# ShengkaiWu/IoU-aware-single-stage-object-detector

Measured on AMD Instinct MI355X. Metric: images/sec at 1333x800, IoU-aware RetinaNet R-50-FPN, higher is better.
Workload: dtype fp32; 1 GPU; IoU-aware RetinaNet R-50-FPN fp32, batch 8 per GPU, 3x800x1344 (1333x800 padded to /32), random-init weights, whole inference path incl. NMS, device-to-host copy and bbox2result (the reference's simple_test: per-class arrays on the host; batch i's host part runs under batch i+1's device part, the last one inside the timed region); global_batch=8, parallelism=dp1, dets_per_image=100

## Files before the change

### include/iouaware.h

```cpp
#ifndef IOUAWARE_H
#define IOUAWARE_H

#include <stddef.h>
#include <stdint.h>

#ifdef __cplusplus
extern "C" {
#endif

#define IA_MAX_LEVELS 8
#define IA_MAX_ANCHORS 16
#define IA_MAX_NMS_PRE 4096
#define IA_MAX_CANDIDATES 8192
#define IA_MAX_PER_IMG 1024

#define IA_F32 0
#define IA_BF16 1
#define IA_F16 2
#define IA_F64 3

#define IA_LAYOUT_NCHW 0
#define IA_LAYOUT_NHWC 1

#define IA_CLS_SIGMOID 0
// ... 120 lines not shown
    int32_t H[IA_MAX_LEVELS], W[IA_MAX_LEVELS];
} ia_wino_geom;
typedef struct {
    int32_t c0, n;
    int32_t dst_channels, dst_offset;
    float *dst[IA_MAX_LEVELS];
} ia_wino_seg;
int ia_wino_tiles(const ia_wino_geom *g, int32_t *tiles);
int ia_wino_input_transform(const ia_wino_geom *g, const float *const *x, int channels, int groups,
                            const float *pre_scale, const float *pre_shift, int pre_relu, float *V,
                            void *stream);
int ia_wino_output_transform(const ia_wino_geom *g, const float *M, int channels, int groups,
                             const float *bias, int relu, int nseg, const ia_wino_seg *segs,
                             void *stream);
int ia_wino_mid_transform(const ia_wino_geom *g, const float *M, int channels, int groups_m,
                          const float *bias, int relu, float *V, int groups_v, void *stream);
int ia_wino_in_gemm(const ia_wino_geom *g, const float *const *x, int channels, const float *pre_scale,
                    const float *pre_shift, int pre_relu, const float *u_packed, float *M, void *stream);
int ia_wino_conv3x3_c64(const ia_wino_geom *g, const float *const *x, int channels, const float *pre_scale,
                        const float *pre_shift, int pre_relu, const float *u_packed, const float *bias,
                        int relu, float *const *y, void *stream);

int ia_wino_grad_output_transform(const ia_wino_geom *g, const float *const *dy, int channels,
                                  float *dM, void *stream);

#define IA_COLSUM_MAX_STRIPS 512
size_t ia_relu_bwd_bias_grad_workspace_bytes(int64_t rows, int n);
int ia_wino_weight_transform(const float *w, int n_in, int n_out, int64_t stride_in,
                             int64_t stride_out, int64_t stride_ky, int64_t stride_kx, int flip,
                             const double *G, float *U, void *stream);
int ia_wino_weight_grad(const float *dU, int n_in, int n_out, const double *G, float *dW,
                        int64_t stride_in, int64_t stride_out, int64_t stride_ky, int64_t stride_kx,
                        void *stream);
int ia_bn_fold_fwd(const float *w, const float *gamma, const float *beta, const float *mean,
                   const float *inv_std, int cout, int K, float *w_out, float *b_out, void *stream);
int ia_bn_fold_bwd(const float *dw_folded, const float *db_folded, const float *w, const float *gamma,
                   const float *mean, const float *inv_std, int cout, int K, float *dw,
                   float *dgamma, float *dbeta, void *stream);
int ia_relu_bwd_bias_grad(const float *dy, const float *y, int64_t rows, int n, float *g, float *db,
                          void *workspace, size_t workspace_bytes, void *stream);

int ia_linear_bias_act(const float *A, const float *W, const float *bias, const float *residual,
                       float *D, int64_t rows, int k, int n, int relu, void *workspace,
                       size_t workspace_bytes, void *stream);
int ia_linear_bias_act_bf16(const void *A, const void *W, const float *bias, const void *residual,
                            void *D, int64_t rows, int k, int n, int relu, void *workspace,
                            size_t workspace_bytes, void *stream);
int ia_batched_gemm(const float *A, const float *W, float *D, int batch, int64_t rows, int k, int n,
                    void *workspace, size_t workspace_bytes, void *stream);
int ia_batched_gemm_stream(const float *A, const float *W, float *D, int batch, int64_t rows, int k,
                           int n, void *stream);
int ia_batched_gemm_split3(const float *V, const void *U3, float *D, int batch, int64_t rows, int k,
                           int n, void *stream);

size_t ia_im2col3x3_bytes(int B, int H, int W, int C, int stride, int dtype);
int ia_im2col3x3_nhwc(const void *x, void *col, int B, int H, int W, int C, int stride, int dtype,
                      void *stream);
int ia_conv1x1_strided(const void *x, const void *W_kn, const float *bias, const void *residual,
                       void *D, int B, int H, int W, int k, int n, int stride, int relu, int dtype,
                       void *workspace, size_t workspace_bytes, void *stream);
int ia_col2im3x3_nhwc(const void *dcol, void *dx, int B, int H, int W, int C, int stride, int dtype,
                      void *stream);

size_t ia_deform_im2col3x3_bytes(int B, int H, int W, int C, int stride, int pad, int dil);
int ia_deform_im2col3x3_nhwc(const float *x, const float *offset, int64_t offset_pix_stride,
                             const float *mask, int64_t mask_pix_stride, int mask_logits,
                             float *col, int B, int H, int W, int C, int stride, int pad,
                             int dil, int deformable_groups, void *stream);
int ia_deform_col2im3x3_nhwc(const float *dcol, const float *x, const float *offset,
                             int64_t offset_pix_stride, const float *mask,
                             int64_t mask_pix_stride, float *dx, float *d_offset, float *d_mask,
                             int B, int H, int W, int C, int stride, int pad, int dil,
                             int deformable_groups, void *stream);

int ia_gemm_tuning(int mode);

int ia_gemm_table_add(int64_t m, int64_t n, int64_t k, int flags, int batch, int dtype,
                      int solution_index);
int ia_gemm_table_clear(void);
int ia_gemm_table_dump(int64_t *rows7, int capacity);
int ia_gemm_table_stats(int64_t *hits_misses_stale);
int ia_gemm_library_version(void);

int ia_linear_bias_act_wt(const float *A, const float *W_nk, const float *bias,
                          const float *residual, float *D, int64_t rows, int k, int n, int relu,
                          void *workspace, size_t workspace_bytes, void *stream);
int ia_gemm_tn(const float *G, const float *X, float *D, int batch, int64_t rows, int n, int k,
               void *workspace, size_t workspace_bytes, void *stream);


int ia_focal_loss_fwd(const void *cls, int dtype, const int64_t *labels,
                      const float *label_weights, int B, int A, int C, int HW, float gamma,
                      float alpha, double *loss_sum, void *stream);
int ia_focal_loss_bwd(const void *cls, int dtype, const int64_t *labels,
                      const float *label_weights, int B, int A, int C, int HW, float gamma,
                      float alpha, float gscale, const float *gscale_dev, float *grad_cls,
                      void *stream);

int ia_smooth_l1_fwd(const void *pred, int dtype, const float *target, const float *weight,
                     int B, int A, int HW, float beta, double *loss_sum, void *stream);
int ia_smooth_l1_bwd(const void *pred, int dtype, const float *target, const float *weight,
                     int B, int A, int HW, float beta, float gscale, const float *gscale_dev,
                     float *grad_pred, void *stream);

int ia_balanced_l1_fwd(const void *pred, int dtype, const float *target, const float *weight,
                       int B, int A, int HW, float beta, float alpha, float gamma, double *loss_sum,
// ... 386 lines not shown
```

### iou-aware-single-stage-object-detector_amd/csrc/wino_split_gemm.hip

```cpp
#include "ia_internal.hpp"

namespace ia {

typedef __attribute__((ext_vector_type(8))) __bf16 bf16x8;
typedef __attribute__((ext_vector_type(16))) float f32x16;

constexpr int kSgBM = 128;
constexpr int kSgBN = 128;
constexpr int kSgBK = 32;
constexpr int kSgThreads = 256;
constexpr int kSgImg = 64 * 16;
constexpr int kSgStage = 2 * 4 * 3 * kSgImg;

struct SplitGemmArgs {
    const float *v;
    const uint4 *up;
    float *d;
    int64_t rows;
    int K, N, np32;
    int ntiles, mtiles;
};

__device__ __forceinline__ void split3(const float4 &x0, const float4 &x1, bf16x8 &h, bf16x8 &m, bf16x8 &l)
{
    const float x[8] = {x0.x, x0.y, x0.z, x0.w, x1.x, x1.y, x1.z, x1.w};
#pragma unroll
    for (int e = 0; e < 8; ++e) {
        const __bf16 hb = (__bf16)x[e];
        const float r = x[e] - (float)hb;
        const __bf16 mb = (__bf16)r;
        h[e] = hb;
        m[e] = mb;
        l[e] = (__bf16)(r - (float)mb);
    }
}

__global__ void __launch_bounds__(kSgThreads, 2) k_gemm_split3(SplitGemmArgs a)
{
    __shared__ __attribute__((aligned(16))) unsigned char s_a[kSgStage];
    __shared__ __attribute__((aligned(16))) unsigned char s_b[kSgStage];
    const int tid = threadIdx.x, lane = tid & 63, wv = tid >> 6;
    const int wm = wv >> 1, wn = wv & 1;
    int nt, b;
    int64_t row0;
    {
        const int total = (int)gridDim.x, q = total >> 3, r = total & 7;
        const int xcd = (int)blockIdx.x & 7, idx = (int)blockIdx.x >> 3;
        int t = xcd < r ? xcd * (q + 1) + idx : r * (q + 1) + (xcd - r) * q + idx;
        nt = t % a.ntiles;
        t /= a.ntiles;
        row0 = (int64_t)(t % a.mtiles) * kSgBM;
        b = t / a.mtiles;
    }
    const int nchunk = a.K / kSgBK;

    int64_t r = row0 + wv * 32 + (lane & 31);
    if (r >= a.rows) r = a.rows - 1;
    const float *vp = a.v + ((int64_t)b * a.rows + r) * a.K + 8 * (lane >> 5);
    const uint4 *up = a.up + ((int64_t)b * (a.K / 16) * a.np32 + nt * 4) * (3 * 64);
    const int64_t ks_stride = (int64_t)a.np32 * 3 * 64;

    float4 x0, x1, x2, x3;
    uint4 u0, u1, u2, u3, u4, u5;
#define SG_LOAD(c)                                                                                  \
    {                                                                                               \
        const float *src = vp + (c) * kSgBK;                                                        \
        x0 = *reinterpret_cast<const float4 *>(src);                                                \
        x1 = *reinterpret_cast<const float4 *>(src + 4);                                            \
        x2 = *reinterpret_cast<const float4 *>(src + 16);                                           \
        x3 = *reinterpret_cast<const float4 *>(src + 20);                                           \
        const uint4 *us = up + (int64_t)(2 * (c)) * ks_stride;                                      \
        u0 = us[tid];                                                                               \
        u1 = us[tid + 256];                                                                         \
// ... 54 lines not shown
                }
#pragma unroll
            for (int i = 0; i < 2; ++i)
#pragma unroll
                for (int j = 0; j < 2; ++j)
                    hi[i][j] = __builtin_amdgcn_mfma_f32_32x32x16_bf16(fa[i][0], fb[j][0], hi[i][j], 0, 0, 0);
#pragma unroll
            for (int i = 0; i < 2; ++i)
#pragma unroll
                for (int j = 0; j < 2; ++j)
                    lo[i][j] = __builtin_amdgcn_mfma_f32_32x32x16_bf16(fa[i][1], fb[j][1], lo[i][j], 0, 0, 0);
#pragma unroll
            for (int i = 0; i < 2; ++i)
#pragma unroll
                for (int j = 0; j < 2; ++j)
                    lo[i][j] = __builtin_amdgcn_mfma_f32_32x32x16_bf16(fa[i][0], fb[j][2], lo[i][j], 0, 0, 0);
#pragma unroll
            for (int i = 0; i < 2; ++i)
#pragma unroll
                for (int j = 0; j < 2; ++j)
                    lo[i][j] = __builtin_amdgcn_mfma_f32_32x32x16_bf16(fa[i][2], fb[j][0], lo[i][j], 0, 0, 0);
#pragma unroll
            for (int i = 0; i < 2; ++i)
#pragma unroll
                for (int j = 0; j < 2; ++j)
                    lo[i][j] = __builtin_amdgcn_mfma_f32_32x32x16_bf16(fa[i][0], fb[j][1], lo[i][j], 0, 0, 0);
#pragma unroll
            for (int i = 0; i < 2; ++i)
#pragma unroll
                for (int j = 0; j < 2; ++j)
                    lo[i][j] = __builtin_amdgcn_mfma_f32_32x32x16_bf16(fa[i][1], fb[j][0], lo[i][j], 0, 0, 0);
        }
    }
#undef SG_LOAD
#undef SG_STORE

    float *dst = a.d + (int64_t)b * a.rows * a.N;
#pragma unroll
    for (int j = 0; j < 2; ++j) {
        const int col = nt * kSgBN + wn * 64 + j * 32 + (lane & 31);
        if (col >= a.N) continue;
#pragma unroll
        for (int i = 0; i < 2; ++i) {
            const int64_t rb = row0 + wm * 64 + i * 32 + 4 * (lane >> 5);
#pragma unroll
            for (int e = 0; e < 16; ++e) {
                const int64_t row = rb + (e & 3) + 8 * (e >> 2);
                if (row < a.rows) dst[row * a.N + col] = hi[i][j][e] + lo[i][j][e];
            }
        }
    }
}

}

extern "C" int ia_batched_gemm_split3(const float *V, const void *U3, float *D, int batch, int64_t rows, int k,
                                      int n, void *stream)
{
    if (!V || !U3 || !D || rows < 1 || batch < 1 || batch > 65535 || k < ia::kSgBK || k % ia::kSgBK || n < 1)
        return IA_E_ARG;
    if (((uintptr_t)V & 15u) || ((uintptr_t)U3 & 15u) || ((uintptr_t)D & 3u)) return IA_E_ARG;
    const int64_t mt = (rows + ia::kSgBM - 1) / ia::kSgBM, ntiles = (n + ia::kSgBN - 1) / ia::kSgBN;
    if (mt * ntiles * batch > 2147483647LL) return IA_E_ARG;
    ia::SplitGemmArgs a;
    a.v = V; a.up = (const uint4 *)U3; a.d = D; a.rows = rows; a.K = k; a.N = n;
    a.np32 = (int)(ntiles * (ia::kSgBN / 32));
    a.ntiles = (int)ntiles; a.mtiles = (int)mt;
    const dim3 grid((unsigned)(mt * ntiles * batch)), block(ia::kSgThreads);
    hipLaunchKernelGGL(ia::k_gemm_split3, grid, block, 0, (hipStream_t)stream, a);
    return ia::hip_status(hipGetLastError());
}
```

### iou-aware-single-stage-object-detector_amd/iouaware/_lib.py

```python
import ctypes as C
import os

IA_MAX_LEVELS = 8
IA_MAX_ANCHORS = 16
IA_MAX_NMS_PRE = 4096
IA_MAX_CANDIDATES = 8192
IA_MAX_PER_IMG = 1024
IA_F32, IA_BF16, IA_F16, IA_F64 = 0, 1, 2, 3
IA_LAYOUT_NCHW, IA_LAYOUT_NHWC = 0, 1
IA_CLS_SIGMOID, IA_CLS_SOFTMAX = 0, 1
IA_CLS_SIGMOID_NOIOU, IA_CLS_SOFTMAX_NOIOU = 2, 3
IA_LOSS_SLOTS = 64
IA_MAX_TARGET_BATCH = 16
IA_GN_CHUNK = 256

_CSRC = os.path.join(os.path.dirname(os.path.abspath(__file__)), '..', 'csrc')
SO_PATH = os.path.abspath(os.path.join(_CSRC, 'libiouaware_hip.so'))


class HeadGeom(C.Structure):
    _fields_ = [('num_levels', C.c_int32), ('num_anchors', C.c_int32),
                ('num_classes', C.c_int32), ('nms_pre', C.c_int32),
                ('H', C.c_int32 * IA_MAX_LEVELS), ('W', C.c_int32 * IA_MAX_LEVELS),
                ('stride', C.c_int32 * IA_MAX_LEVELS),
# ... 110 lines not shown
    'ia_select_topk': (_i, [_G, _vp, _i, _vp, _vp, _sz, _vp]),
    'ia_decode_fuse_rowmax_grouped': (_i, [_G, _P, _i, _i, _vp, _vp, _sz, _vp]),
    'ia_select_topk_grouped': (_i, [_G, _vp, _i, _vp, _vp, _sz, _vp]),
    'ia_decode_stage': (_i, [_G, _P, _i, _i, _vp, _vp, _i, _vp, _sz, _vp]),
    'ia_get_bboxes_status_offset': (_sz, [_G, _i]),
    'ia_debug_fused_spin_limit': (_i, [_i64]),
    'ia_profile_stage_events': (_i, [_vp, _vp]),
    'ia_gather_decode': (_i, [_G, _P, _i, _i, _vp, _vp, _vp, _i, _vp, _vp, _vp, _vp]),
    'ia_multiclass_nms_workspace_bytes': (_sz, [_i, _i, _i]),
    'ia_multiclass_nms': (_i, [_vp, _vp, _vp, _i, _i, _i, _f, _f, _i, _vp, _sz, _vp, _vp, _vp,
                               _vp, _vp, _vp, _vp]),
    'ia_multiclass_soft_nms_workspace_bytes': (_sz, [_i, _i, _i]),
    'ia_multiclass_soft_nms': (_i, [_vp, _vp, _i, _i, _i, _f, _f, _i, _f, _f, _i, _vp, _sz, _vp, _vp,
                                    _vp, _vp, _vp, _vp, _vp]),
    'ia_soft_nms': (_i, [_vp, _i, _f, _i, _f, _f, _vp, _vp, _vp, _vp]),
    'ia_get_bboxes_workspace_bytes': (_sz, [_G, _i]),
    'ia_get_bboxes': (_i, [_G, _P, _i, _i, _vp, _vp, _i, _f, _f, _i, _vp, _sz, _vp, _vp, _vp,
                           _vp, _vp]),
    'ia_multiclass_nms_lazy_workspace_bytes': (_sz, [_i, _i, _i]),
    'ia_multiclass_nms_lazy': (_i, [_vp, _vp, _vp, _i, _i, _i, _f, _f, _i, _i, _vp, _sz, _vp, _vp, _vp,
                                    _vp, _vp]),
    'ia_get_bboxes_lazy': (_i, [_G, _P, _i, _i, _vp, _vp, _i, _f, _f, _i, _i, _vp, _sz, _vp, _vp, _vp,
                                _vp, _vp]),
    'ia_get_bboxes_workspace_layout': (_i, [_G, _i, C.POINTER(_sz * 8)]),
    'ia_nms_workspace_bytes': (_sz, [_i]),
    'ia_nms': (_i, [_vp, _i, _f, _vp, _vp, _vp, _sz, _vp]),
    'ia_nms_f64_workspace_bytes': (_sz, [_i]),
    'ia_nms_f64': (_i, [_vp, _i, _f, _vp, _vp, _vp, _sz, _vp]),
    'ia_image_transform': (_i, [C.POINTER(ImageDesc), _i, C.POINTER(C.c_float), C.POINTER(C.c_float),
                                _i, _i, _i, _i, _vp, _vp]),
    'ia_wino_tiles': (_i, [C.POINTER(WinoGeom), C.POINTER(C.c_int32)]),
    'ia_wino_input_transform': (_i, [C.POINTER(WinoGeom), C.POINTER(C.c_void_p), _i, _i, _vp, _vp, _i,
                                     _vp, _vp]),
    'ia_wino_grad_output_transform': (_i, [C.POINTER(WinoGeom), C.POINTER(C.c_void_p), _i, _vp, _vp]),
    'ia_wino_weight_transform': (_i, [_vp, _i, _i, C.c_int64, C.c_int64, C.c_int64, C.c_int64, _i,
                                      C.POINTER(C.c_double), _vp, _vp]),
    'ia_wino_weight_grad': (_i, [_vp, _i, _i, C.POINTER(C.c_double), _vp, C.c_int64, C.c_int64,
                                 C.c_int64, C.c_int64, _vp]),
    'ia_bn_fold_fwd': (_i, [_vp, _vp, _vp, _vp, _vp, _i, _i, _vp, _vp, _vp]),
    'ia_bn_fold_bwd': (_i, [_vp, _vp, _vp, _vp, _vp, _vp, _i, _i, _vp, _vp, _vp, _vp]),
    'ia_relu_bwd_bias_grad_workspace_bytes': (C.c_size_t, [C.c_int64, _i]),
    'ia_relu_bwd_bias_grad': (_i, [_vp, _vp, C.c_int64, _i, _vp, _vp, _vp, C.c_size_t, _vp]),
    'ia_wino_output_transform': (_i, [C.POINTER(WinoGeom), _vp, _i, _i, _vp, _i, _i,
                                      C.POINTER(WinoSeg), _vp]),
    'ia_wino_mid_transform': (_i, [C.POINTER(WinoGeom), _vp, _i, _i, _vp, _i, _vp, _i, _vp]),
    'ia_wino_in_gemm': (_i, [C.POINTER(WinoGeom), C.POINTER(C.c_void_p), _i, _vp, _vp, _i, _vp, _vp, _vp]),
    'ia_wino_conv3x3_c64': (_i, [C.POINTER(WinoGeom), C.POINTER(C.c_void_p), _i, _vp, _vp, _i, _vp, _vp, _i,
                                 C.POINTER(C.c_void_p), _vp]),
    'ia_linear_bias_act': (_i, [_vp, _vp, _vp, _vp, _vp, _i64, _i, _i, _i, _vp, _sz, _vp]),
    'ia_linear_bias_act_bf16': (_i, [_vp, _vp, _vp, _vp, _vp, _i64, _i, _i, _i, _vp, _sz, _vp]),
    'ia_batched_gemm': (_i, [_vp, _vp, _vp, _i, _i64, _i, _i, _vp, _sz, _vp]),
    'ia_batched_gemm_stream': (_i, [_vp, _vp, _vp, _i, _i64, _i, _i, _vp]),
    'ia_batched_gemm_split3': (_i, [_vp, _vp, _vp, _i, _i64, _i, _i, _vp]),
    'ia_linear_bias_act_wt': (_i, [_vp, _vp, _vp, _vp, _vp, _i64, _i, _i, _i, _vp, _sz, _vp]),
    'ia_gemm_tuning': (_i, [_i]),
    'ia_im2col3x3_bytes': (_sz, [_i, _i, _i, _i, _i, _i]),
    'ia_im2col3x3_nhwc': (_i, [_vp, _vp, _i, _i, _i, _i, _i, _i, _vp]),
    'ia_col2im3x3_nhwc': (_i, [_vp, _vp, _i, _i, _i, _i, _i, _i, _vp]),
    'ia_deform_im2col3x3_bytes': (_sz, [_i, _i, _i, _i, _i, _i, _i]),
    'ia_deform_im2col3x3_nhwc': (_i, [_vp, _vp, _i64, _vp, _i64, _i, _vp, _i, _i, _i, _i, _i, _i, _i, _i, _vp]),
    'ia_deform_col2im3x3_nhwc': (_i, [_vp, _vp, _vp, _i64, _vp, _i64, _vp, _vp, _vp, _i, _i, _i, _i, _i, _i,
                                      _i, _i, _vp]),
    'ia_conv1x1_strided': (_i, [_vp, _vp, _vp, _vp, _vp, _i, _i, _i, _i, _i, _i, _i, _i, _vp, _sz, _vp]),
    'ia_gemm_table_add': (_i, [_i64, _i64, _i64, _i, _i, _i, _i]),
    'ia_gemm_table_clear': (_i, []),
    'ia_gemm_table_dump': (_i, [_vp, _i]),
    'ia_gemm_table_stats': (_i, [_vp]),
    'ia_gemm_library_version': (_i, []),
    'ia_gemm_tn': (_i, [_vp, _vp, _vp, _i, _i64, _i, _i, _vp, _sz, _vp]),
    'ia_focal_loss_fwd': (_i, [_vp, _i, _vp, _vp, _i, _i, _i, _i, _f, _f, _vp, _vp]),
    'ia_focal_loss_bwd': (_i, [_vp, _i, _vp, _vp, _i, _i, _i, _i, _f, _f, _f, _vp, _vp, _vp]),
    'ia_smooth_l1_fwd': (_i, [_vp, _i, _vp, _vp, _i, _i, _i, _f, _vp, _vp]),
    'ia_smooth_l1_bwd': (_i, [_vp, _i, _vp, _vp, _i, _i, _i, _f, _f, _vp, _vp, _vp]),
    'ia_balanced_l1_fwd': (_i, [_vp, _i, _vp, _vp, _i, _i, _i, _f, _f, _f, _vp, _vp]),
    'ia_balanced_l1_bwd': (_i, [_vp, _i, _vp, _vp, _i, _i, _i, _f, _f, _f, _f, _vp, _vp, _vp]),
    'ia_focal_loss_balanced_fwd': (_i, [_vp, _i, _vp, _vp, _vp, _i, _i, _i, _i, _f, _f, _f, _vp, _vp]),
    'ia_focal_loss_balanced_bwd': (_i, [_vp, _i, _vp, _vp, _vp, _i, _i, _i, _i, _f, _f, _f, _vp, _f,
                                        _vp, _vp, _vp]),
    'ia_smooth_l1_balanced_fwd': (_i, [_vp, _i, _vp, _vp, _vp, _i, _i, _i, _f, _f, _vp, _vp]),
    'ia_smooth_l1_balanced_bwd': (_i, [_vp, _i, _vp, _vp, _vp, _i, _i, _i, _f, _f, _f, _vp, _vp,
                                       _vp]),
    'ia_iou_bce_fwd': (_i, [_G, _i, _vp, _vp, _i, _vp, _vp, _i, _vp, _vp, _vp]),
    'ia_iou_bce_bwd': (_i, [_G, _i, _vp, _vp, _i, _vp, _vp, _i, _f, _vp, _vp, _vp, _vp]),
    'ia_anchor_targets': (_i, [_G, _vp, _vp, _vp, _i, _i, _vp, _f, _f, _f, _f, _vp, _vp, _vp, _vp,
                               _vp, _vp, _vp]),
    'ia_anchor_targets_ptrs': (_i, [_G, C.POINTER(C.c_void_p), C.POINTER(C.c_void_p),
                                    C.POINTER(C.c_int32), _i, C.POINTER(C.c_int32), _f, _f, _f, _f,
                                    _vp, _vp, _vp, _vp, _vp, _vp, _vp]),
    'ia_head_loss_workspace_bytes': (_sz, [_G, _i]),
    'ia_head_loss_workspace_bytes_cfg': (_sz, [_G, _i, C.POINTER(HeadLossCfg)]),
    'ia_head_loss_fwd': (_i, [_G, _P, _i, _i, C.POINTER(HeadTargets), C.POINTER(HeadLossCfg), _vp,
                              _sz, _vp, _vp]),
    'ia_head_loss_bwd': (_i, [_G, _P, _i, _i, C.POINTER(HeadTargets), C.POINTER(HeadLossCfg), _vp,
                              _vp, _vp, _P, _vp]),
    'ia_head_loss_fwd_nhwc': (_i, [_G, _P, C.POINTER(LevelPixStrides), _i, C.POINTER(HeadTargets),
                                   C.POINTER(HeadLossCfg), _vp, _sz, _vp, _vp]),
    'ia_head_loss_bwd_nhwc': (_i, [_G, _P, C.POINTER(LevelPixStrides), _i, C.POINTER(HeadTargets),
                                   C.POINTER(HeadLossCfg), _vp, _vp, _P, C.POINTER(LevelPixStrides),
                                   _vp]),
    'ia_head_loss_fwd_box': (_i, [_G, _P, _i, _i, C.POINTER(HeadTargets), C.POINTER(HeadLossCfg),
                                  C.POINTER(BoxLossCfg), _vp, _sz, _vp, _vp]),
    'ia_head_loss_bwd_box': (_i, [_G, _P, _i, _i, C.POINTER(HeadTargets), C.POINTER(HeadLossCfg),
                                  C.POINTER(BoxLossCfg), _vp, _vp, _vp, _P, _vp]),
    'ia_head_loss_fwd_nhwc_box': (_i, [_G, _P, C.POINTER(LevelPixStrides), _i, C.POINTER(HeadTargets),
                                       C.POINTER(HeadLossCfg), C.POINTER(BoxLossCfg), _vp, _sz, _vp, _vp]),
    'ia_head_loss_bwd_nhwc_box': (_i, [_G, _P, C.POINTER(LevelPixStrides), _i, C.POINTER(HeadTargets),
# ... 136 lines not shown
```

### iou-aware-single-stage-object-detector_amd/iouaware/winograd.py

```python
import collections
import ctypes as C

import numpy as np
import torch

from . import _lib
from .ops import _ptr, _stream, stream_id

_G = np.array([[1 / 4, 0, 0], [-1 / 6, -1 / 6, -1 / 6], [-1 / 6, 1 / 6, -1 / 6],
               [1 / 24, 1 / 12, 1 / 6], [1 / 24, -1 / 12, 1 / 6], [0, 0, 1]], dtype=np.float64)


_G_DEV = {}


def transform_weight(w):
    if w.dim() != 4 or w.shape[2] != 3 or w.shape[3] != 3:
        raise ValueError('Winograd F(4,3) needs a 3x3 kernel, got %s' % (tuple(w.shape),))
    g = w.detach().to(torch.float64)
    G = _G_DEV.get(g.device)
    if G is None:
        G = _G_DEV[g.device] = torch.from_numpy(_G).to(g.device)
    u = torch.einsum('ik,ockl,jl->ijco', G, g, G)
    return u.reshape(36, g.shape[1], g.shape[0]).to(torch.float32).contiguous()
# ... 74 lines not shown
def _timed(kind, nbytes, launch):
    if TIMING is None:
        return launch()
    e0, e1 = torch.cuda.Event(enable_timing=True), torch.cuda.Event(enable_timing=True)
    e0.record()
    launch()
    e1.record()
    TIMING.append((kind, e0, e1, nbytes))


def input_transform(plan, xs, groups, out, pre=None):
    ptrs = (C.c_void_p * len(xs))(*[x.data_ptr() for x in xs])
    ps, pb, pr = pre if pre is not None else (None, None, False)
    ch = int(xs[0].shape[1])
    _timed('in', plan.T * ch * 4 * (16 + 36), lambda: _lib.check(
        _lib.lib().ia_wino_input_transform(C.byref(plan.geom), ptrs, ch, int(groups), _ptr(ps),
                                           _ptr(pb), int(bool(pr)), _ptr(out), _stream()),
        'ia_wino_input_transform'))
    return out


def output_transform(plan, m, channels, groups, bias, relu, segments):
    segs = (_lib.WinoSeg * len(segments))()
    for k, (c0, n, dst, off) in enumerate(segments):
        segs[k].c0, segs[k].n = int(c0), int(n)
        segs[k].dst_channels, segs[k].dst_offset = int(dst[0].shape[1]), int(off)
        for l, t in enumerate(dst):
            segs[k].dst[l] = t.data_ptr()
    _timed('out', plan.T * int(channels) * 4 * (36 + 16), lambda: _lib.check(
        _lib.lib().ia_wino_output_transform(C.byref(plan.geom), _ptr(m), int(channels), int(groups),
                                            _ptr(bias), int(bool(relu)), len(segments), segs,
                                            _stream()), 'ia_wino_output_transform'))


MID_CHANNELS = 32


def mid_transform(plan, m, channels, groups_m, bias, relu, out, groups_v):
    _timed('mid', plan.T * int(channels) * 4 * (36 + 36), lambda: _lib.check(
        _lib.lib().ia_wino_mid_transform(C.byref(plan.geom), _ptr(m), int(channels), int(groups_m),
                                         _ptr(bias), int(bool(relu)), _ptr(out), int(groups_v),
                                         _stream()), 'ia_wino_mid_transform'))
    return out


_LT_WS_BYTES = 128 << 20


STREAM_BMM = True
_STREAM_BMM_SHAPES = ((64, 64),)


SPLIT_GEMM = True
_SPLIT_SHAPES = ((256, 720),)


def split3_pack_u(u):
    b, k, n = u.shape
    if k % 32:
        raise ValueError('the split GEMM needs K in multiples of 32')
    npad = (n + 127) // 128 * 128
    u = u.to(torch.float32)
    h = u.to(torch.bfloat16)
    r = u - h.float()
    m = r.to(torch.bfloat16)
    lo = (r - m.float()).to(torch.bfloat16)
    p = torch.zeros((b, 3, k, npad), dtype=torch.bfloat16, device=u.device)
    p[:, 0, :, :n], p[:, 1, :, :n], p[:, 2, :, :n] = h, m, lo
    return p.view(b, 3, k // 16, 2, 8, npad // 32, 32).permute(0, 2, 5, 1, 3, 6, 4).contiguous() \
            .view(b, k // 16, npad // 32, 3, 64, 8)


def split_shape(u):
    return (int(u.shape[1]), int(u.shape[2])) in _SPLIT_SHAPES


def batched_gemm(v, u, out, u3=None):
    from . import ops
    ops._ensure_gemm_table()
    batch, rows, k = v.shape
    n = u.shape[2]
    if not (v.is_contiguous() and u.is_contiguous() and out.is_contiguous()):
        raise ValueError('batched_gemm needs contiguous stacks')
    if SPLIT_GEMM and u3 is not None and (k, n) in _SPLIT_SHAPES and v.dtype == torch.float32:
        if u3.dtype != torch.bfloat16 or tuple(u3.shape) != (batch, k // 16, (n + 127) // 128 * 4, 3, 64, 8) \
                or not u3.is_contiguous():
            raise ValueError('u3 is not split3_pack_u of this U')
        _lib.check(_lib.lib().ia_batched_gemm_split3(_ptr(v), _ptr(u3), _ptr(out), int(batch), int(rows),
                                                     int(k), int(n), _stream()), 'ia_batched_gemm_split3')
        return out
    if STREAM_BMM and (k, n) in _STREAM_BMM_SHAPES and rows >= 4096 and v.dtype == torch.float32:
        _lib.check(_lib.lib().ia_batched_gemm_stream(_ptr(v), _ptr(u), _ptr(out), int(batch), int(rows),
                                                     int(k), int(n), _stream()), 'ia_batched_gemm_stream')
        return out
    ws = _scratch(v.device, 'lt_ws', (_LT_WS_BYTES // 4,))
    _lib.check(_lib.lib().ia_batched_gemm(_ptr(v), _ptr(u), _ptr(out), int(batch), int(rows), int(k),
                                          int(n), _ptr(ws), _LT_WS_BYTES, _stream()),
               'ia_batched_gemm')
    return out


FUSE_IN_GEMM = True
FUSE_OUT = True
_IN_GEMM_CHANNELS = (64,)


def pack_u_fragments(u):
    b, k, n = u.shape
    if k % 16 or n % 16:
        raise ValueError('fragment order needs multiples of 16 channels')
    return u.reshape(b, k // 16, 4, 4, n // 16, 16).permute(0, 4, 1, 2, 5, 3).contiguous() \
            .view(b, n // 16, k // 16, 64, 4)


def input_transform_gemm(plan, xs, u_packed, out, pre=None, epilogue=None):
    ptrs = (C.c_void_p * len(xs))(*[x.data_ptr() for x in xs])
    ps, pb, pr = pre if pre is not None else (None, None, False)
    if epilogue is not None:
        bias, relu, ys = epilogue
        if out is not None or len(ys) != len(xs):
            raise ValueError('the one-launch form writes ys, one per level, and no M')
        yptrs = (C.c_void_p * len(ys))(*[y.data_ptr() for y in ys])
        _lib.check(_lib.lib().ia_wino_conv3x3_c64(C.byref(plan.geom), ptrs, int(xs[0].shape[1]), _ptr(ps),
                                                  _ptr(pb), int(bool(pr)), _ptr(u_packed), _ptr(bias),
                                                  int(bool(relu)), yptrs, _stream()),
                   'ia_wino_conv3x3_c64')
        return ys
    _lib.check(_lib.lib().ia_wino_in_gemm(C.byref(plan.geom), ptrs, int(xs[0].shape[1]), _ptr(ps), _ptr(pb),
                                          int(bool(pr)), _ptr(u_packed), _ptr(out), _stream()),
               'ia_wino_in_gemm')
    return out


class WinogradConv3x3(object):

    def __init__(self, weight, bias, relu=False):
        self.u = transform_weight(weight)
        self.u_packed = None
        if self.u.shape[1] == self.u.shape[2] and self.u.shape[1] in _IN_GEMM_CHANNELS:
            self.u_packed = pack_u_fragments(self.u)
        self.bias = None if bias is None else bias.detach().to(torch.float32).contiguous()
        self.relu = relu
        self.cin, self.cout = self.u.shape[1], self.u.shape[2]
        if self.cout % 4:
            raise ValueError('output channels must be a multiple of 4')
        self._plans = collections.OrderedDict()

    def usable(self, x):
        return _usable(x) and x.shape[1] == self.cin \
            and not (torch.is_grad_enabled() and x.requires_grad)
# ... 29 lines not shown
    n_pad = (na + nb + granule - 1) // granule * granule
    dev = a.weight.device
    u = torch.zeros((36, F, n_pad), dtype=torch.float32, device=dev)
    u[:, :, :na] = transform_weight(a.weight)
    bias = torch.zeros(n_pad, dtype=torch.float32, device=dev)
    bias[:na] = a.bias.detach().float()
    if b is not None:
        u[:, :, na:na + nb] = transform_weight(b.weight)
        bias[na:na + nb] = b.bias.detach().float()
    return u.contiguous(), bias.contiguous(), na, nb


class _WinogradTowers(object):

    FUSE_MID = True
    mid_bias = None
    u0_3 = None
    u_3 = None

    def __init__(self, head):
        convs_c, convs_r = list(head.cls_convs), list(head.reg_convs)
        self.n_layers = len(convs_c)
        F = head.feat_channels
        if head.in_channels % 4 or F % 4:
            raise ValueError('channel counts must be multiples of 4')
        self.F, self.cin = F, head.in_channels
        self.u0 = torch.cat([transform_weight(convs_c[0].conv.weight),
                             transform_weight(convs_r[0].conv.weight)], dim=2).contiguous()
        self.u = [torch.cat([transform_weight(convs_c[i].conv.weight),
                             transform_weight(convs_r[i].conv.weight)], dim=0).contiguous()
                  for i in range(1, self.n_layers)]
        self._plans = collections.OrderedDict()

    def usable(self, feats):
        return all(_usable(x) and x.shape[1] == self.cin for x in feats) \
            and not torch.is_grad_enabled()

    def _towers(self, feats):
        B, dev = feats[0].shape[0], feats[0].device
        sizes = [tuple(x.shape[-2:]) for x in feats]
        key = (B, tuple(sizes), dev, stream_id())
        plan = _plan_for(self._plans, key, lambda: _Plan(sizes, B, dev))
        T, F = plan.T, self.F
        u3 = (lambda i: self.u_3[i]) if self.u_3 is not None else (lambda i: None)
        v = input_transform(plan, feats, 1, plan.buf('v', (36, T, self.cin)))
        m = batched_gemm(v, self.u0, plan.buf('m', (36, T, 2 * F)), self.u0_3)
        new = lambda c: [torch.empty((B, c, h, w), dtype=torch.float32, device=dev,
                                     memory_format=torch.channels_last) for (h, w) in sizes]
        if self.FUSE_MID and self.mid_bias is not None and F % MID_CHANNELS == 0:
            groups = 1
            for i, u in enumerate(self.u):
                v = mid_transform(plan, m, 2 * F, groups, self.mid_bias[i], True,
                                  plan.buf('v', (72, T, F)), 2)
                m = batched_gemm(v, u, plan.buf('m', (72, T, F)), u3(i))
                groups = 2
            v = mid_transform(plan, m, 2 * F, groups, self.mid_bias[self.n_layers - 1], True,
                              plan.buf('v', (72, T, F)), 2)
            return plan, v, new
        acts = plan.acts('a', 2 * F)
        self._layer_out(plan, m, 1, 0, acts)
        for i, u in enumerate(self.u):
            v = input_transform(plan, acts, 2, plan.buf('v', (72, T, F)))
            m = batched_gemm(v, u, plan.buf('m', (72, T, F)), u3(i))
            nxt = plan.acts('b' if acts is plan.acts('a', 2 * F) else 'a', 2 * F)
            self._layer_out(plan, m, 2, i + 1, nxt)
            acts = nxt
        v = input_transform(plan, acts, 2, plan.buf('v', (72, T, F)))
        return plan, v, new

    @staticmethod
    def _out_conv(plan, v, name, u, bias, segments, u3=None):
        n = u.shape[2]
        m = batched_gemm(v, u, plan.buf(name, (36, plan.T, n)), u3)
        output_transform(plan, m, n, 1, bias, False, segments)


class WinogradHead(_WinogradTowers):

    def __init__(self, head):
        convs_c, convs_r = list(head.cls_convs), list(head.reg_convs)
        if any(m.with_norm or not m.with_activatation for m in convs_c + convs_r):
            raise NotImplementedError('towers with norm layers / without ReLU')
        super(WinogradHead, self).__init__(head)

        def bias(m):
            conv = m.conv
            b = conv.bias if conv.bias is not None else torch.zeros(conv.out_channels,
                                                                     device=conv.weight.device)
            return b.detach().float()

        self.b = [torch.cat([bias(mc), bias(mr)]).contiguous() for mc, mr in zip(convs_c, convs_r)]
        self.mid_bias = self.b
        if head.retina_cls.out_channels % 4:
            raise ValueError('A*C must be a multiple of 4')
        self.u_cls, self.b_cls, self.c_cls, _ = _pair(head.retina_cls, None, self.F, 1)
        self.u_ri, self.b_ri, self.c_reg, self.c_iou = _pair(head.retina_reg, head.retina_iou,
                                                             self.F, 16)
        pack = lambda u: split3_pack_u(u) if split_shape(u) else None
        self.u0_3 = pack(self.u0)
        self.u_3 = [pack(u) for u in self.u]
        self.u_cls3 = pack(self.u_cls)

    def _layer_out(self, plan, m, groups, i, acts):
        output_transform(plan, m, 2 * self.F, groups, self.b[i], True, [(0, 2 * self.F, acts, 0)])

    def __call__(self, feats):
        plan, v, new = self._towers(feats)
        cls, reg, iou = new(self.c_cls), new(self.c_reg), new(self.c_iou)
        self._out_conv(plan, v[:36], 'mc', self.u_cls, self.b_cls, [(0, self.c_cls, cls, 0)], self.u_cls3)
        self._out_conv(plan, v[36:], 'mr', self.u_ri, self.b_ri,
                       [(0, self.c_reg, reg, 0), (self.c_reg, self.c_iou, iou, 0)])
        return cls, reg, iou


class WinogradFCOSHead(_WinogradTowers):

    def __init__(self, head):
        convs_c, convs_r = list(head.cls_convs), list(head.reg_convs)
        for m in convs_c + convs_r:
            if not (m.with_norm and m.norm_cfg.get('type') == 'GN' and m.with_activatation
                    and m.conv.bias is None and m.activate_last and plain_3x3(m.conv)):
                raise NotImplementedError('FCOS towers other than 3x3 conv (no bias) + GN + ReLU')
        super(WinogradFCOSHead, self).__init__(head)
        self.groups = 2 * int(convs_c[0].norm.num_groups)
        self.eps = float(convs_c[0].norm.eps)
        if any(float(m.norm.eps) != self.eps or 2 * int(m.norm.num_groups) != self.groups
               for m in convs_c + convs_r):
            raise NotImplementedError('towers with different GroupNorm settings')
        self.gn = [(torch.cat([mc.norm.weight.detach(), mr.norm.weight.detach()]).float().contiguous(),
                    torch.cat([mc.norm.bias.detach(), mr.norm.bias.detach()]).float().contiguous())
                   for mc, mr in zip(convs_c, convs_r)]
        self.u_cc, self.b_cc, self.c_cls, self.c_ctr = _pair(head.fcos_cls, head.fcos_centerness,
                                                             self.F, 16)
        self.u_ri, self.b_ri, self.c_reg, self.c_iou = _pair(head.fcos_reg,
                                                             getattr(head, 'fcos_iou', None),
                                                             self.F, 16)
        if self.c_reg % 4:
            raise ValueError('the regression output needs a multiple of 4 channels')
        self.scales = torch.stack([s.scale.detach().float() for s in head.scales]).contiguous()
        self.calls = 0

    def usable(self, feats):
        return len(feats) <= self.scales.numel() and super(WinogradFCOSHead, self).usable(feats)

    def _layer_out(self, plan, m, groups, i, acts):
        from .fcos_ops import groupnorm_relu_
        output_transform(plan, m, 2 * self.F, groups, None, False, [(0, 2 * self.F, acts, 0)])
        g, b = self.gn[i]
        groupnorm_relu_(acts, g, b, self.groups, self.eps, relu=True)

    def __call__(self, feats):
        plan, v, new = self._towers(feats)
        cls, ctr, reg = new(self.c_cls), new(self.c_ctr), new(self.c_reg)
# ... 16 lines not shown
```

Baseline: 426.7 img/s.

## Add persistent double-buffered split-bf16 GEMM and route cls tower layers through it

Adds a persistent, XCD-aware tile-scheduled split3 bf16 MFMA GEMM kernel. It uses direct global-to-LDS loads with double buffering, so the next tile's first chunk is prefetched while the current one computes. This kernel becomes the default when K spans at least two chunks. The (256,256) shape is added to the split path, and the cls-tower half of the 72-batch mid-layer GEMMs (first 36) now runs on the split kernel while the reg half stays on the library GEMM. This aims to cut load latency and launch-tail cost, at the cost of inline asm, m0 juggling and an extra launch per layer.

```diff
diff --git a/include/iouaware.h b/include/iouaware.h
--- a/include/iouaware.h
+++ b/include/iouaware.h
@@ -196,6 +196,8 @@
                            int n, void *stream);
 int ia_batched_gemm_split3(const float *V, const void *U3, float *D, int batch, int64_t rows, int k,
                            int n, void *stream);
+int ia_batched_gemm_split3_variant(const float *V, const void *U3, float *D, int batch, int64_t rows,
+                                   int k, int n, void *stream, int variant);
 
 size_t ia_im2col3x3_bytes(int B, int H, int W, int C, int stride, int dtype);
 int ia_im2col3x3_nhwc(const void *x, void *col, int B, int H, int W, int C, int stride, int dtype,
diff --git a/iou-aware-single-stage-object-detector_amd/csrc/wino_split_gemm.hip b/iou-aware-single-stage-object-detector_amd/csrc/wino_split_gemm.hip
--- a/iou-aware-single-stage-object-detector_amd/csrc/wino_split_gemm.hip
+++ b/iou-aware-single-stage-object-detector_amd/csrc/wino_split_gemm.hip
@@ -19,6 +19,7 @@
     int64_t rows;
     int K, N, np32;
     int ntiles, mtiles;
+    int batch;
 };
 
 __device__ __forceinline__ void split3(const float4 &x0, const float4 &x1, bf16x8 &h, bf16x8 &m, bf16x8 &l)
@@ -179,21 +180,210 @@
     }
 }
 
-}
-
-extern "C" int ia_batched_gemm_split3(const float *V, const void *U3, float *D, int batch, int64_t rows, int k,
-                                      int n, void *stream)
+constexpr int kSpImgA = 2 * 4 * 2;
+constexpr int kSpImgB = 2 * 4 * 3;
+constexpr int kSpStage = (kSpImgA + kSpImgB) * kSgImg;
+
+typedef __attribute__((address_space(3))) unsigned char lds_byte;
+
+__device__ __forceinline__ void glds16(const void *src, unsigned char *dst)
+{
+    const unsigned lds = __builtin_amdgcn_readfirstlane((unsigned)(size_t)(lds_byte *)dst);
+    unsigned keep;
+    asm volatile("s_mov_b32 %0, m0\n\ts_mov_b32 m0, %2\n\ts_nop 0\n\tglobal_load_lds_dwordx4 %1, off\n\ts_mov_b32 m0, %0"
+                 : "=&s"(keep) : "v"(src), "s"(lds) : "memory");
+}
+
+struct SpTile {
+    int nt, b;
+    int64_t row0;
+};
+
+__device__ __forceinline__ SpTile sp_tile(const SplitGemmArgs &a, int slot, int total)
+{
+    SpTile t;
+    const int q = total >> 3, r8 = total & 7;
+    const int xcd = slot & 7, idx = slot >> 3;
+    int i = xcd < r8 ? xcd * (q + 1) + idx : r8 * (q + 1) + (xcd - r8) * q + idx;
+    t.nt = i % a.ntiles;
+    i /= a.ntiles;
+    t.row0 = (int64_t)(i % a.mtiles) * kSgBM;
+    t.b = i / a.mtiles;
+    return t;
+}
+
+__device__ __forceinline__ void sp_stage(const SplitGemmArgs &a, const SpTile &t, int c, int wv, int lane,
+                                         unsigned char *st)
+{
+    int64_t row = t.row0 + wv * 32 + (lane & 31);
+    if (row >= a.rows) row = a.rows - 1;
+    const float *vp = a.v + ((int64_t)t.b * a.rows + row) * a.K + c * kSgBK + 8 * (lane >> 5);
+#pragma unroll
+    for (int s = 0; s < 2; ++s)
+#pragma unroll
+        for (int h = 0; h < 2; ++h)
+            glds16(vp + 16 * s + 4 * h, st + ((s * 4 + wv) * 2 + h) * kSgImg);
+    const int64_t ks_stride = (int64_t)a.np32 * 3 * 64;
+    const uint4 *up = a.up + (((int64_t)t.b * (a.K / 16) + 2 * c) * a.np32 + t.nt * 4) * (3 * 64) + lane;
+#pragma unroll
+    for (int i = 0; i < 6; ++i) {
+        const int s = i / 3, j = wv + 4 * (i % 3);
+        glds16(up + s * ks_stride + j * 64, st + (kSpImgA + s * 12 + j) * kSgImg);
+    }
+}
+
+__global__ void __launch_bounds__(kSgThreads, 2) k_gemm_split_pipe(SplitGemmArgs a)
+{
+    __shared__ __attribute__((aligned(16))) unsigned char s_ab[2 * kSpStage];
+    const int tid = threadIdx.x, lane = tid & 63, wv = __builtin_amdgcn_readfirstlane(tid >> 6);
+    const int wm = wv >> 1, wn = wv & 1;
+    const int total = a.ntiles * a.mtiles * a.batch, G = (int)gridDim.x;
+    const int nchunk = a.K / kSgBK;
+
+    int slot = (int)blockIdx.x;
+    SpTile cur = sp_tile(a, slot, total);
+    sp_stage(a, cur, 0, wv, lane, s_ab);
+    int g = 0;
+    for (;;) {
+        const bool more = slot + G < total;
+        SpTile nxt = cur;
+        if (more) nxt = sp_tile(a, slot + G, total);
+
+        f32x16 hi[2][2], lo[2][2];
+#pragma unroll
+        for (int i = 0; i < 2; ++i)
+#pragma unroll
+            for (int j = 0; j < 2; ++j)
+#pragma unroll
+                for (int e = 0; e < 16; ++e) {
+                    hi[i][j][e] = 0.0f;
+                    lo[i][j][e] = 0.0f;
+                }
+
+        for (int c = 0; c < nchunk; ++c, ++g) {
+            asm volatile("s_waitcnt vmcnt(0)" ::: "memory");
+            __syncthreads();
+            unsigned char *other = s_ab + ((g + 1) & 1) * kSpStage;
+            if (c + 1 < nchunk)
+                sp_stage(a, cur, c + 1, wv, lane, other);
+            else if (more)
+                sp_stage(a, nxt, 0, wv, lane, other);
+            const unsigned char *sa = s_ab + (g & 1) * kSpStage, *sb = sa + kSpImgA * kSgImg;
+#pragma unroll
+            for (int s = 0; s < 2; ++s) {
+                bf16x8 fa[2][3], fb[2][3];
+#pragma unroll
+                for (int i = 0; i < 2; ++i) {
+                    const unsigned char *pa = sa + ((s * 4 + wm * 2 + i) * 2 * 64 + lane) * 16;
+                    const float4 x0 = *reinterpret_cast<const float4 *>(pa);
+                    const float4 x1 = *reinterpret_cast<const float4 *>(pa + kSgImg);
+                    split3(x0, x1, fa[i][0], fa[i][1], fa[i][2]);
+#pragma unroll
+                    for (int p = 0; p < 3; ++p)
+                        fb[i][p] = *reinterpret_cast<const bf16x8 *>(sb + (((s * 4 + wn * 2 + i) * 3 + p) * 64 + lane) * 16);
+                }
+#pragma unroll
+                for (int i = 0; i < 2; ++i)
+#pragma unroll
+                    for (int j = 0; j < 2; ++j)
+                        hi[i][j] = __builtin_amdgcn_mfma_f32_32x32x16_bf16(fa[i][0], fb[j][0], hi[i][j], 0, 0, 0);
+#pragma unroll
+                for (int i = 0; i < 2; ++i)
+#pragma unroll
+                    for (int j = 0; j < 2; ++j)
+                        lo[i][j] = __builtin_amdgcn_mfma_f32_32x32x16_bf16(fa[i][1], fb[j][1], lo[i][j], 0, 0, 0);
+#pragma unroll
+                for (int i = 0; i < 2; ++i)
+#pragma unroll
+                    for (int j = 0; j < 2; ++j)
+                        lo[i][j] = __builtin_amdgcn_mfma_f32_32x32x16_bf16(fa[i][0], fb[j][2], lo[i][j], 0, 0, 0);
+#pragma unroll
+                for (int i = 0; i < 2; ++i)
+#pragma unroll
+                    for (int j = 0; j < 2; ++j)
+                        lo[i][j] = __builtin_amdgcn_mfma_f32_32x32x16_bf16(fa[i][2], fb[j][0], lo[i][j], 0, 0, 0);
+#pragma unroll
+                for (int i = 0; i < 2; ++i)
+#pragma unroll
+                    for (int j = 0; j < 2; ++j)
+                        lo[i][j] = __builtin_amdgcn_mfma_f32_32x32x16_bf16(fa[i][0], fb[j][1], lo[i][j], 0, 0, 0);
+#pragma unroll
+                for (int i = 0; i < 2; ++i)
+#pragma unroll
+                    for (int j = 0; j < 2; ++j)
+                        lo[i][j] = __builtin_amdgcn_mfma_f32_32x32x16_bf16(fa[i][1], fb[j][0], lo[i][j], 0, 0, 0);
+            }
+        }
+
+        int el = lane, n = a.N;
+        asm volatile("" : "+v"(el), "+s"(n));
+        const int col = cur.nt * kSgBN + wn * 64 + (el & 31);
+        float *dst = a.d + ((int64_t)cur.b * a.rows + cur.row0 + wm * 64) * n + cur.nt * kSgBN + wn * 64;
+        const int lane_off = 4 * (el >> 5) * n + (el & 31);
+        const int lrow = wm * 64 + 4 * (el >> 5);
+        const int nrows = (int)min((int64_t)kSgBM, a.rows - cur.row0);
+#pragma unroll
+        for (int j = 0; j < 2; ++j) {
+            if (col + j * 32 >= n) continue;
+#pragma unroll
+            for (int i = 0; i < 2; ++i)
+#pragma unroll
+                for (int e = 0; e < 16; ++e) {
+                    const int k = i * 32 + (e & 3) + 8 * (e >> 2);
+                    if (nrows == kSgBM || lrow + k < nrows) dst[lane_off + k * n + j * 32] = hi[i][j][e] + lo[i][j][e];
+                }
+        }
+        if (!more) break;
+        cur = nxt;
+        slot += G;
+    }
+}
+
+}
+
+static int cu_count()
+{
+    static int cus[64];
+    int dev = 0;
+    if (hipGetDevice(&dev) != hipSuccess || dev < 0 || dev >= 64) return 256;
+    if (!cus[dev]) {
+        int c = 0;
+        if (hipDeviceGetAttribute(&c, hipDeviceAttributeMultiprocessorCount, dev) != hipSuccess || c < 4) c = 256;
+        cus[dev] = c;
+    }
+    return cus[dev];
+}
+
+extern "C" int ia_batched_gemm_split3_variant(const float *V, const void *U3, float *D, int batch, int64_t rows,
+                                              int k, int n, void *stream, int variant)
 {
     if (!V || !U3 || !D || rows < 1 || batch < 1 || batch > 65535 || k < ia::kSgBK || k % ia::kSgBK || n < 1)
         return IA_E_ARG;
     if (((uintptr_t)V & 15u) || ((uintptr_t)U3 & 15u) || ((uintptr_t)D & 3u)) return IA_E_ARG;
+    if (variant < -1 || variant > 1 || n > (1 << 24)) return IA_E_ARG;
     const int64_t mt = (rows + ia::kSgBM - 1) / ia::kSgBM, ntiles = (n + ia::kSgBN - 1) / ia::kSgBN;
-    if (mt * ntiles * batch > 2147483647LL) return IA_E_ARG;
+    const int64_t total = mt * ntiles * batch;
+    if (total > 2147483647LL) return IA_E_ARG;
     ia::SplitGemmArgs a;
     a.v = V; a.up = (const uint4 *)U3; a.d = D; a.rows = rows; a.K = k; a.N = n;
     a.np32 = (int)(ntiles * (ia::kSgBN / 32));
-    a.ntiles = (int)ntiles; a.mtiles = (int)mt;
-    const dim3 grid((unsigned)(mt * ntiles * batch)), block(ia::kSgThreads);
-    hipLaunchKernelGGL(ia::k_gemm_split3, grid, block, 0, (hipStream_t)stream, a);
+    a.ntiles = (int)ntiles; a.mtiles = (int)mt; a.batch = batch;
+    if (variant < 0) variant = (k >= 2 * ia::kSgBK && rows >= ia::kSgBM && 3 * n > ntiles * ia::kSgBN) ? 1 : 0;
+    int64_t g = total;
+    if (variant == 1) {
+        const int64_t cap = (2 * cu_count()) / 8 * 8;
+        if (cap >= 8 && g > cap) g = cap;
+    }
+    const dim3 grid((unsigned)g), block(ia::kSgThreads);
+    if (variant == 0)
+        hipLaunchKernelGGL(ia::k_gemm_split3, grid, block, 0, (hipStream_t)stream, a);
+    else
+        hipLaunchKernelGGL(ia::k_gemm_split_pipe, grid, block, 0, (hipStream_t)stream, a);
     return ia::hip_status(hipGetLastError());
 }
+
+extern "C" int ia_batched_gemm_split3(const float *V, const void *U3, float *D, int batch, int64_t rows, int k,
+                                      int n, void *stream)
+{
+    return ia_batched_gemm_split3_variant(V, U3, D, batch, rows, k, n, stream, -1);
+}
diff --git a/iou-aware-single-stage-object-detector_amd/iouaware/_lib.py b/iou-aware-single-stage-object-detector_amd/iouaware/_lib.py
--- a/iou-aware-single-stage-object-detector_amd/iouaware/_lib.py
+++ b/iou-aware-single-stage-object-detector_amd/iouaware/_lib.py
@@ -186,6 +186,7 @@
     'ia_batched_gemm': (_i, [_vp, _vp, _vp, _i, _i64, _i, _i, _vp, _sz, _vp]),
     'ia_batched_gemm_stream': (_i, [_vp, _vp, _vp, _i, _i64, _i, _i, _vp]),
     'ia_batched_gemm_split3': (_i, [_vp, _vp, _vp, _i, _i64, _i, _i, _vp]),
+    'ia_batched_gemm_split3_variant': (_i, [_vp, _vp, _vp, _i, _i64, _i, _i, _vp, _i]),
     'ia_linear_bias_act_wt': (_i, [_vp, _vp, _vp, _vp, _vp, _i64, _i, _i, _i, _vp, _sz, _vp]),
     'ia_gemm_tuning': (_i, [_i]),
     'ia_im2col3x3_bytes': (_sz, [_i, _i, _i, _i, _i, _i]),
diff --git a/iou-aware-single-stage-object-detector_amd/iouaware/winograd.py b/iou-aware-single-stage-object-detector_amd/iouaware/winograd.py
--- a/iou-aware-single-stage-object-detector_amd/iouaware/winograd.py
+++ b/iou-aware-single-stage-object-detector_amd/iouaware/winograd.py
@@ -150,7 +150,7 @@
 
 
 SPLIT_GEMM = True
-_SPLIT_SHAPES = ((256, 720),)
+_SPLIT_SHAPES = ((256, 256), (256, 720))
 
 
 def split3_pack_u(u):
@@ -173,7 +173,7 @@
     return (int(u.shape[1]), int(u.shape[2])) in _SPLIT_SHAPES
 
 
-def batched_gemm(v, u, out, u3=None):
+def batched_gemm(v, u, out, u3=None, nsplit=None):
     from . import ops
     ops._ensure_gemm_table()
     batch, rows, k = v.shape
@@ -181,19 +181,27 @@
     if not (v.is_contiguous() and u.is_contiguous() and out.is_contiguous()):
         raise ValueError('batched_gemm needs contiguous stacks')
     if SPLIT_GEMM and u3 is not None and (k, n) in _SPLIT_SHAPES and v.dtype == torch.float32:
-        if u3.dtype != torch.bfloat16 or tuple(u3.shape) != (batch, k // 16, (n + 127) // 128 * 4, 3, 64, 8) \
-                or not u3.is_contiguous():
+        ns = batch if nsplit is None else int(nsplit)
+        if u3.dtype != torch.bfloat16 or not 0 < ns <= batch \
+                or tuple(u3.shape) != (ns, k // 16, (n + 127) // 128 * 4, 3, 64, 8) or not u3.is_contiguous():
             raise ValueError('u3 is not split3_pack_u of this U')
-        _lib.check(_lib.lib().ia_batched_gemm_split3(_ptr(v), _ptr(u3), _ptr(out), int(batch), int(rows),
+        _lib.check(_lib.lib().ia_batched_gemm_split3(_ptr(v), _ptr(u3), _ptr(out), int(ns), int(rows),
                                                      int(k), int(n), _stream()), 'ia_batched_gemm_split3')
+        if ns < batch:
+            _library_gemm(v[ns:], u[ns:], out[ns:])
         return out
     if STREAM_BMM and (k, n) in _STREAM_BMM_SHAPES and rows >= 4096 and v.dtype == torch.float32:
         _lib.check(_lib.lib().ia_batched_gemm_stream(_ptr(v), _ptr(u), _ptr(out), int(batch), int(rows),
                                                      int(k), int(n), _stream()), 'ia_batched_gemm_stream')
         return out
+    return _library_gemm(v, u, out)
+
+
+def _library_gemm(v, u, out):
+    batch, rows, k = v.shape
     ws = _scratch(v.device, 'lt_ws', (_LT_WS_BYTES // 4,))
     _lib.check(_lib.lib().ia_batched_gemm(_ptr(v), _ptr(u), _ptr(out), int(batch), int(rows), int(k),
-                                          int(n), _ptr(ws), _LT_WS_BYTES, _stream()),
+                                          int(u.shape[2]), _ptr(ws), _LT_WS_BYTES, _stream()),
                'ia_batched_gemm')
     return out
 
@@ -329,7 +337,7 @@
             for i, u in enumerate(self.u):
                 v = mid_transform(plan, m, 2 * F, groups, self.mid_bias[i], True,
                                   plan.buf('v', (72, T, F)), 2)
-                m = batched_gemm(v, u, plan.buf('m', (72, T, F)), u3(i))
+                m = batched_gemm(v, u, plan.buf('m', (72, T, F)), u3(i), 36)
                 groups = 2
             v = mid_transform(plan, m, 2 * F, groups, self.mid_bias[self.n_layers - 1], True,
                               plan.buf('v', (72, T, F)), 2)
@@ -338,7 +346,7 @@
         self._layer_out(plan, m, 1, 0, acts)
         for i, u in enumerate(self.u):
             v = input_transform(plan, acts, 2, plan.buf('v', (72, T, F)))
-            m = batched_gemm(v, u, plan.buf('m', (72, T, F)), u3(i))
+            m = batched_gemm(v, u, plan.buf('m', (72, T, F)), u3(i), 36)
             nxt = plan.acts('b' if acts is plan.acts('a', 2 * F) else 'a', 2 * F)
             self._layer_out(plan, m, 2, i + 1, nxt)
             acts = nxt
@@ -375,7 +383,7 @@
                                                              self.F, 16)
         pack = lambda u: split3_pack_u(u) if split_shape(u) else None
         self.u0_3 = pack(self.u0)
-        self.u_3 = [pack(u) for u in self.u]
+        self.u_3 = [pack(u[:36]) for u in self.u]
         self.u_cls3 = pack(self.u_cls)
 
     def _layer_out(self, plan, m, groups, i, acts):
```

After: 426.6 img/s. No clear change (-0.0%).
